# xuhao1/TaichiSLAM

Measured on AMD Instinct MI355X. Metric: depth-frames/s integrated (640x480->512^3 TSDF), higher is better.
Workload: dtype f16 storage / f32 + int64 fixed-point arithmetic; 1 GPU; BASELINE configs[1]: single 640x480 u16 depth stream (sphere room r=3 m, 1 deg/frame) -> DenseTSDF 512^3 / 2 cm, recast_step 2, max_ray 5 m; one stream+submap per GPU

## Files before the change

### taichislam_amd/csrc/tsl_integrate.hip

```cpp
#include "tsl_tsdf.hpp"
#include <hip/hip_ext.h>

namespace tsl {

#ifdef TSL_TIMING
#define TSL_T0() const int _wv = (blockIdx.x * (int)blockDim.x + (int)threadIdx.x) >> 6
#define TSL_TICK(F, k) do { long long _n = wall_clock64(); if (lane_id() == 0 && _wv < 16384) (F).dbg[_wv * 16 + (k)] = _n; } while (0)
#else
#define TSL_T0() do {} while (0)
#define TSL_TICK(F, k) do {} while (0)
#endif

#define SCATTER_TILE 4096

struct RayRegs { float pf0, pf1, pf2, d0, d1, d2, P0, P1, P2, w; long long qden; int n; };

__device__ __forceinline__ uint32_t wave_min_u32(uint32_t v)
{
    for (int d = 32; d > 0; d >>= 1) { const uint32_t o = (uint32_t)__shfl_xor((int)v, d); v = o < v ? o : v; }
    return v;
}
__device__ __forceinline__ RayRegs make_ray(const uint4 rec, int n, const FrameParams& P)
{
    RayRegs R;
// ... 527 lines not shown
#else
__device__ __forceinline__ int acc_swz5(int l) { return l ^ (((l >> 8) ^ (l >> 5)) & 31); }
#endif
struct StepK { float vs, rvs, T0, T1, T2; int hN, hNz; };

template <bool FASTDIV>
__device__ __forceinline__ void step_eval(const RayRegs& R, const StepK& K, int j, int* slot, float* qf)
{
    const float jf = (float)j;
    const float x0 = (R.d0 * jf) * K.vs + K.T0, x1 = (R.d1 * jf) * K.vs + K.T1, x2 = (R.d2 * jf) * K.vs + K.T2;
    const int i0 = rnd_i(div_vs(x0, K.vs, K.rvs, FASTDIV ? 1 : 0)), i1 = rnd_i(div_vs(x1, K.vs, K.rvs, FASTDIV ? 1 : 0)), i2 = rnd_i(div_vs(x2, K.vs, K.rvs, FASTDIV ? 1 : 0));
    *slot = acc_swz5((((i0 + K.hN) & 15) << 8) | (((i1 + K.hN) & 15) << 4) | ((i2 + K.hNz) & 15));
    const float v0 = R.P0 - x0, v1 = R.P1 - x1, v2 = R.P2 - x2;
    const float s2 = (v0 * v0 + v1 * v1) + v2 * v2;
    const float dist = sqrt_rn_norm(fmaxf(s2, 1.2621774483536189e-29f));
    const float dot = (v0 * R.pf0 + v1 * R.pf1) + v2 * R.pf2;
    const float sd = dot == 0.0f ? 0.0f : copysignf(dist, dot);
    *qf = rintf((R.w * sd) * TSL_FIX_SCALE);
}

__device__ __forceinline__ bool fits_i32(long long q) { return q == (long long)(int)q; }
__device__ __forceinline__ float from_fix32(long long q) { return (float)(int)q * (float)TSL_FIX_INV; }

#define FLUSH_CHUNK 4
template <int N>
__device__ __forceinline__ void apply_chunk(const uint32_t* old, const long long* qn, const long long* qd, uint32_t* nv, bool all_small)
{
    if (all_small) {
#pragma unroll
        for (int q = 0; q < N; ++q) nv[q] = apply_update_f(old[q], from_fix32(qn[q]), from_fix32(qd[q]));
    } else {
#pragma unroll
        for (int q = 0; q < N; ++q) nv[q] = apply_update_f(old[q], from_fix(qn[q]), from_fix(qd[q]));
    }
}

__device__ __forceinline__ int uni(int v) { return __builtin_amdgcn_readfirstlane(v); }
#define IT_UNIT 0
#define IT_POOL 1
#define IT_SLAB 2
#define IT_NP   3
#define IT_TMALL 4
#define IT_FMASK 5
#define IT_OFF  6
#define IT_N    (IT_OFF + TSL_NB)
#define IT_WORDS (IT_N + TSL_NB + 2)
#define NRANGE (PLAN_NCLS * (TSL_NB + 1))

template <bool TEX, bool FASTDIV, int NT, int SPT, int WPE>
__global__ void __launch_bounds__(NT, WPE) k_integrate_batch(MapDev M, BatchDev B, int kind)
{
    constexpr int CSEGS = SPT * NT, VPT = TSL_BRK3 / NT, CH = VPT < FLUSH_CHUNK ? VPT : FLUSH_CHUNK;
    static_assert(VPT <= 16, "the written / first-touch masks hold 16 voxels per thread");
#ifdef TSL_EXP_SLOT16
    __shared__ ulonglong2 s_acc[TSL_BRK3];
#define S_NUM(i) s_acc[i].x
#define S_DEN(i) s_acc[i].y
#else
    __shared__ unsigned long long s_num[TSL_BRK3];
    __shared__ unsigned long long s_den[TSL_BRK3];
#define S_NUM(i) s_num[i]
#define S_DEN(i) s_den[i]
#endif
    __shared__ unsigned long long s_keys[CSEGS];
    __shared__ uint32_t s_win[TEX ? TSL_BRK3 : 1];
    __shared__ int s_bin[64];
    __shared__ int s_claim[2];
    __shared__ int s_uq[TSL_NB];
    __shared__ int s_cum[NRANGE + 1];
    __shared__ int s_it[3][IT_WORDS];
    uint32_t okmask = 0u;
#pragma unroll
    for (int q = 0; q < TSL_NB; ++q) if (q < B.n) {
        const FrameDev& Fq = B.f[q];
        if (Fq.counters[HDR_FAIL] == 0) okmask |= 1u << q;
        const int nact = min(Fq.counters[1], Fq.max_frame_bricks);
        for (int i = blockIdx.x * NT + threadIdx.x; i < nact; i += gridDim.x * NT) { const int b = Fq.act_b[i]; Fq.bhist[b] = 0; Fq.bcursor[b] = 0; }
    }
    if (threadIdx.x < TSL_NB) s_uq[threadIdx.x] = 0;
    if (threadIdx.x == 0) {
        int acc = 0, k = 0;
#ifdef TSL_CLASS_MAJOR
        for (int c = 0; c < PLAN_NCLS; ++c) {
            s_cum[k++] = acc; acc += min(B.f[0].counters[HDR_UNITS + c], B.f[0].unit_cap);
            for (int q = 0; q < TSL_NB; ++q) { s_cum[k++] = acc; if ((okmask >> q) & 1u) acc += min(B.f[q].counters[HDR_PARTS + c], B.f[q].part_cap); }
        }
#else
        for (int c = 0; c < PLAN_NCLS; ++c) { s_cum[k++] = acc; if (kind != 2) acc += min(B.f[0].counters[HDR_UNITS + c], B.f[0].unit_cap); }
        for (int c = 0; c < PLAN_NCLS; ++c)
            for (int q = 0; q < TSL_NB; ++q) { s_cum[k++] = acc; if (kind != 1 && ((okmask >> q) & 1u)) acc += min(B.f[q].counters[HDR_PARTS + c], B.f[q].part_cap); }
#endif
        s_cum[NRANGE] = acc;
        s_claim[0] = __hip_atomic_fetch_add(&B.f[0].counters[kind == 2 ? HDR_CLAIM2 : HDR_CLAIM], 1, __ATOMIC_RELAXED, __HIP_MEMORY_SCOPE_AGENT);
    }
    __syncthreads();
    const int total = uni(s_cum[NRANGE]);
    int* const claim = &B.f[0].counters[kind == 2 ? HDR_CLAIM2 : HDR_CLAIM];
    auto entry_of = [&](int r, int* kq) -> int4 {
        int k = 0;
#pragma unroll
        for (int j = 1; j < NRANGE; ++j) k += r >= uni(s_cum[j]) ? 1 : 0;
#ifdef TSL_CLASS_MAJOR
// ... 23 lines not shown
            int pool = e.z;
            if (fm == 0u) { fm = 1u; pool = -1; }
            it[IT_UNIT] = kq < 0 ? 1 : 0; it[IT_POOL] = pool; it[IT_SLAB] = kq < 0 ? 0 : e.w; it[IT_NP] = kq < 0 ? 1 : (e.y >> 16) & ((1 << PART_NP_BITS) - 1);
            it[IT_TMALL] = (int)tm; it[IT_FMASK] = (int)fm;
        }
    };
    const int r0 = uni(s_claim[0]);
    if (r0 >= total) return;
    { int kq, io, in; const int4 e = entry_of(r0, &kq); info_of(e, kq, &io, &in); commit(0, e, kq, io, in); }
    __syncthreads();
    auto steps_of = [&](int sl, uint32_t fm) -> int {
        int n = 0;
#pragma unroll
        for (int q = 0; q < TSL_NB; ++q) if ((fm >> q) & 1u) n += max(1, (uni(s_it[sl][IT_N + q]) + CSEGS - 1) / CSEGS);
        return n;
    };
    long long uniq = 0;
    int t = 0, slot = 0, c = 0; (void)t;
    int n_known = 0;
    bool exhausted = false;
    int f = __builtin_ctz((uint32_t)uni(s_it[0][IT_FMASK]));

    unsigned long long kk[SPT]; uint4 recs[SPT]; uint32_t wids[SPT];
#define TSL_SORT_DEAL(KIN, NSEG, FD)                                                                                    \
    {                                                                                                                   \
        int rr[SPT];                                                                                                    \
        _Pragma("unroll") for (int q = 0; q < SPT; ++q) {                                                               \
            const int i = q * NT + (int)threadIdx.x; rr[q] = -1;                                                        \
            if (i < (NSEG)) rr[q] = atomicAdd(&s_bin[63 - (int)(KIN[q] & 63ull)], 1);                                   \
        }                                                                                                               \
        __syncthreads();                                                                                                \
        if (threadIdx.x < 64) {                                                                                         \
            const int cb = s_bin[threadIdx.x]; int inc = cb;                                                            \
            for (int d = 1; d < 64; d <<= 1) { const int o = __shfl_up(inc, d); if ((int)threadIdx.x >= d) inc += o; }  \
            s_bin[threadIdx.x] = inc - cb;                                                                              \
        }                                                                                                               \
        __syncthreads();                                                                                                \
        _Pragma("unroll") for (int q = 0; q < SPT; ++q) if (rr[q] >= 0) s_keys[s_bin[63 - (int)(KIN[q] & 63ull)] + rr[q]] = KIN[q]; \
        __syncthreads();                                                                                                \
        _Pragma("unroll") for (int q = 0; q < SPT; ++q) {                                                               \
            const int i = q * NT + ((q & 1) ? NT - 1 - (int)threadIdx.x : (int)threadIdx.x);                            \
            if (i < (NSEG)) {                                                                                           \
                kk[q] = s_keys[i];                                                                                      \
                const int r = (int)((kk[q] >> (SEG_CNT_BITS + SEG_J_BITS)) & ((1u << STG_RAY_BITS) - 1));               \
                recs[q] = (FD).rayA[r];                                                                                 \
                wids[q] = TEX ? (FD).rayFirst[r] + 1u : 0u;                                                             \
            }                                                                                                           \
        }                                                                                                               \
        if (threadIdx.x < 64) s_bin[threadIdx.x] = 0;               \
    }
#define TSL_PRIME(SL, FQ)                                                                                               \
    {                                                                                                                   \
        const FrameDev& F0 = B.f[FQ];                                                                                   \
        const int off0 = uni(s_it[SL][IT_OFF + (FQ)]), nseg0 = min(uni(s_it[SL][IT_N + (FQ)]), CSEGS);                  \
        unsigned long long k0[SPT];                                                                                     \
        _Pragma("unroll") for (int q = 0; q < SPT; ++q) { const int i = q * NT + threadIdx.x; k0[q] = i < nseg0 ? F0.seg_sorted[off0 + i] : 0ull; } \
        TSL_SORT_DEAL(k0, nseg0, F0)                                                                                    \
    }

    {
#ifdef TSL_EXP_SLOT16
        for (int i = threadIdx.x; i < TSL_BRK3; i += NT) s_acc[i] = make_ulonglong2(0ull, 0ull);
#else
        ulonglong2* zn = reinterpret_cast<ulonglong2*>(s_num); ulonglong2* zd = reinterpret_cast<ulonglong2*>(s_den);
        for (int i = threadIdx.x; i < TSL_BRK3 / 2; i += NT) { zn[i] = make_ulonglong2(0ull, 0ull); zd[i] = make_ulonglong2(0ull, 0ull); }
#endif
// ... 33 lines not shown
        if (threadIdx.x == 0 && first_step) { _ph[0] = _ph[1] = _ph[2] = _ph[3] = _ph[4] = 0; }
        const long long _ta = wall_clock64();
#endif
        const bool has_next = !last_step || n_known >= 1;
        int fx = f, cx = c + 1, slotx = slot;
        if (last_chunk) {
            cx = 0;
            if (!last_frame) fx = f + 1 + __builtin_ctz(later);
            else if (has_next) { slotx = slot1; fx = __builtin_ctz((uint32_t)uni(s_it[slotx][IT_FMASK])); }
        }
        const FrameDev& Fx = B.f[fx];
        unsigned long long kn[SPT];
        const int offx = uni(s_it[slotx][IT_OFF + fx]) + cx * CSEGS;
        const int nsegn = has_next ? min(CSEGS, uni(s_it[slotx][IT_N + fx]) - cx * CSEGS) : 0;
#pragma unroll
        for (int q = 0; q < SPT; ++q) { const int i = q * NT + threadIdx.x; kn[q] = i < nsegn ? Fx.seg_sorted[offx + i] : 0ull; }
        const uint32_t* const twr = M.tw + (size_t)(p >= 0 ? p : 0) * TSL_BRK3;
        if (first_step) { have_old = false; vmask = 0u; }
        if (!TEX && unit && p >= 0 && first_step) {
#pragma unroll
            for (int q = 0; q < VPT; ++q) old[q] = twr[q * NT + threadIdx.x];
            have_old = true;
        }
#pragma unroll
        for (int q = 0; q < SPT; ++q) {
            const int i = q * NT + ((q & 1) ? NT - 1 - (int)threadIdx.x : (int)threadIdx.x);
            if (i >= nseg) continue;
            const unsigned long long key = kk[q];
            const int cnt = (int)(key & ((1u << SEG_CNT_BITS) - 1)), j0 = (int)((key >> SEG_CNT_BITS) & ((1u << SEG_J_BITS) - 1));
            const RayRegs R = make_ray(recs[q], 0, P);
            const uint32_t wid = wids[q];
#ifndef TSL_EXP_STAGGER
#define TSL_EXP_STAGGER 27
#endif
            int off = ((int)((threadIdx.x * (unsigned)TSL_EXP_STAGGER) & 63u) * cnt) >> 6;
            for (int s = 0; s < cnt; s += 2) {
                const int ja = j0 + off; off = (off + 1 == cnt) ? 0 : off + 1;
                const int jb = j0 + off; off = (off + 1 == cnt) ? 0 : off + 1;
                int la, lb; float qa, qb;
                step_eval<FASTDIV>(R, K, ja, &la, &qa);
                step_eval<FASTDIV>(R, K, jb, &lb, &qb);
                long long na = (long long)(int)qa, nb = (long long)(int)qb;
                if (__builtin_expect(__any(!(fabsf(qa) < 2147483648.0f) || !(fabsf(qb) < 2147483648.0f)), 0)) { na = __float2ll_rn(qa); nb = __float2ll_rn(qb); }
                atomicAdd(&S_NUM(la), (unsigned long long)na);
                atomicAdd(&S_DEN(la), (unsigned long long)R.qden);
                if (TEX) atomicMax(&s_win[la], wid);
                const bool vb = s + 1 < cnt;
#ifdef TSL_EXP_ADDZERO
                atomicAdd(&S_NUM(lb), (unsigned long long)(vb ? nb : 0ll));
                atomicAdd(&S_DEN(lb), (unsigned long long)(vb ? R.qden : 0ll));
// ... 16 lines not shown
        }
        if (has_next) TSL_SORT_DEAL(kn, nsegn, Fx)
        if (fetching) info_of(ne, nkq, &nio, &nin);
#ifdef TSL_TIMING
        const long long _tc = wall_clock64();
        if (threadIdx.x == 0) { _ph[0] += _tb - _ta; _ph[1] += _tc - _tb; _ph[4] += 1; }
#endif
        if (!last_chunk) {
            if (fetching) { commit(n_known == 0 ? slot1 : slot2, ne, nkq, nio, nin); ++n_known; __syncthreads(); }
            ++c; continue;
        }
        if (p >= 0 && threadIdx.x == 0) M.touch[p] = 1;
        if (p >= 0 && unit) {
            uint32_t* tw = M.tw + (size_t)p * TSL_BRK3;
            if (!have_old) {
#pragma unroll
                for (int q = 0; q < VPT; ++q) old[q] = tw[q * NT + threadIdx.x];
                have_old = true;
            }
            if (first_frame) {
#pragma unroll
                for (int q = 0; q < VPT; ++q) vmask |= ((old[q] >> 16) == 0u ? 1u : 0u) << (16 + q);
            }
#pragma unroll
            for (int h = 0; h < VPT; h += CH) {
                long long qn[CH], qd[CH]; uint32_t nv[CH]; bool small = true, anyu = false;
#pragma unroll
                for (int q = 0; q < CH; ++q) {
                    const int ls = acc_swz5((h + q) * NT + threadIdx.x);
                    qn[q] = (long long)S_NUM(ls); qd[q] = (long long)S_DEN(ls); S_NUM(ls) = 0ull; S_DEN(ls) = 0ull;
                    small = small && fits_i32(qn[q]) && fits_i32(qd[q]); anyu = anyu || qd[q] != 0;
                }
                if (!__any(anyu)) continue;
                apply_chunk<CH>(old + h, qn, qd, nv, __all(small));
#pragma unroll
                for (int q = 0; q < CH; ++q) {
                    const bool upd = qd[q] != 0;
                    old[h + q] = upd ? nv[q] : old[h + q];
                    vmask |= (upd ? 1u : 0u) << (h + q);
                    uniq += upd ? 1 : 0;
                    if (TEX && upd) {
                        const int l = (h + q) * NT + threadIdx.x;
                        reinterpret_cast<uint2*>(M.col)[(size_t)p * TSL_BRK3 + l] = F.colpix[s_win[acc_swz5(l)] - 1u];
                    }
                }
            }
            if (TEX) for (int i = threadIdx.x; i < TSL_BRK3; i += NT) s_win[i] = 0u;
            if (last_frame) {
                int8_t* obs = M.obs + (size_t)p * TSL_BRK3;
#pragma unroll
                for (int q = 0; q < VPT; ++q) {
                    const int l = q * NT + threadIdx.x;
                    if ((vmask >> q) & 1u) {
                        tw[l] = old[q];
                        if ((vmask >> (16 + q)) & 1u) obs[l] = 1;
                    }
                }
            }
        } else if (p >= 0) {
            ulonglong2* acc = reinterpret_cast<ulonglong2*>(F.acc) + (size_t)rk * TSL_BRK3;
#pragma unroll
            for (int q = 0; q < VPT; ++q) {
                const int l = q * NT + threadIdx.x, ls = acc_swz5(l);
                acc[l] = make_ulonglong2(S_NUM(ls), S_DEN(ls));
                S_NUM(ls) = 0ull; S_DEN(ls) = 0ull;
                if (TEX) { F.accw[(size_t)rk * TSL_BRK3 + l] = s_win[ls]; s_win[ls] = 0u; }
            }
// ... 10 lines not shown
        const long long _td = wall_clock64();
#endif
        {
            const long long u = wave_sum_ll(uniq);
            if (lane_id() == 0 && u) atomicAdd(&s_uq[f], (int)u);
            uniq = 0;
        }
        if (fetching) { commit(n_known == 0 ? slot1 : slot2, ne, nkq, nio, nin); ++n_known; }
#ifdef TSL_TIMING
        if (threadIdx.x == 0 && last_step) _rec[4] = wall_clock64();
        if (threadIdx.x == 0) { _ph[2] += _td - _tc; _ph[3] += wall_clock64() - _td; }
#endif
        if (!has_next && n_known == 0) break;
        __syncthreads();
        c = 0;
        if (last_frame) { ++t; slot = slot1; --n_known; f = __builtin_ctz((uint32_t)uni(s_it[slot][IT_FMASK])); }
        else f = fx;
        if (!has_next) TSL_PRIME(slot, f)
    }
#undef TSL_PRIME
#undef TSL_SORT_DEAL
    __syncthreads();
    if (threadIdx.x < TSL_NB && s_uq[threadIdx.x]) atomic_add_i64(&B.f[threadIdx.x].stats->unique, (long long)s_uq[threadIdx.x]);
}

#ifndef APPLY_SPLIT
#define APPLY_SPLIT 8
#endif
#ifndef APPLY_ROUND
#define APPLY_ROUND 2
#endif
template <bool TEX>
__global__ void __launch_bounds__(256) k_apply_slab(MapDev M, BatchDev B)
{
    __shared__ int s_uq[TSL_NB];
    constexpr int VP = TSL_BRK3 / APPLY_SPLIT / 256;
    uint32_t okmask = 0u;
#pragma unroll
    for (int q = 0; q < TSL_NB; ++q) if (q < B.n && B.f[q].counters[HDR_FAIL] == 0) okmask |= 1u << q;
    const int nheavy = min(B.f[0].counters[HDR_HEAVY], B.f[0].max_frame_bricks);
    const ulonglong2* const slab = reinterpret_cast<const ulonglong2*>(B.f[0].acc);
    if (threadIdx.x < TSL_NB) s_uq[threadIdx.x] = 0;
    __syncthreads();
    for (int item = blockIdx.x; item < nheavy * APPLY_SPLIT; item += gridDim.x) {
        const int4 e = B.f[0].heavy_tab[item / APPLY_SPLIT];
        const int b = e.x, p = e.y;
// ... 83 lines not shown
int launch_segments(tsl_tsdf* m, const BatchDev& B, const FrameParams* hp, int total, hipStream_t st)
{
    const FrameParams& P = hp[0];
    if (P.variant != 2) return TSL_OK;
    const int iblocks = (int)(((int64_t)total * P.split + 255) / 256);
    prof_begin(m, TSL_K_SEGMENTS, st);
    if (P.group) hipLaunchKernelGGL(k_segments<true>, dim3(iblocks, B.n), dim3(256), 0, st, m->M, B);
    else hipLaunchKernelGGL(k_segments<false>, dim3(iblocks, B.n), dim3(256), 0, st, m->M, B);
    prof_end(m, st);
    int unit_max = m->unit_max <= m->unit_floor ? m->unit_max : std::max(m->unit_floor, (int)((long long)m->unit_max * B.n / TSL_NB));
    int unit_half = std::min(unit_max, m->unit_half <= 2048 ? m->unit_half : std::max(2048, (int)((long long)m->unit_half * B.n / TSL_NB)));
    if (P.seq && m->seq_impl) unit_max = unit_half = 1 << 30;
    prof_begin(m, TSL_K_BIN, st);
    hipLaunchKernelGGL(k_plan, dim3((B.f[0].max_frame_bricks + 255) / 256, B.n), dim3(256), 0, st, m->M, B, m->chunks * m->wg * m->spt, unit_max, unit_half);
    hipLaunchKernelGGL(k_scatter, dim3(256, B.n), dim3(256), 0, st, B);
    prof_end(m, st);
    return TSL_OK;
}

int launch_brick(tsl_tsdf* m, const BatchDev& B, const FrameParams& P, int kind, hipStream_t st, hipEvent_t start, hipEvent_t stop)
{
    const int bg = kind == 2 ? m->pgrid : (B.n <= 2 ? (m->bgrid + 1) / 2 : (kind == 1 ? m->ugrid : m->bgrid));
#define TSL_LAUNCH_IB(TEXV, FD) do { \
        if (m->wg == 512 && m->spt == 2 && !TEXV) hipExtLaunchKernelGGL((k_integrate_batch<false, FD, 512, 2, 4>), dim3((2 * m->ncu * bg + 99) / 100), dim3(512), 0, st, start, stop, 0, m->M, B, kind); \
        else if (m->wg == 512) hipExtLaunchKernelGGL((k_integrate_batch<TEXV, FD, 512, 4, 2>), dim3((m->ncu * bg + 99) / 100), dim3(512), 0, st, start, stop, 0, m->M, B, kind); \
        else hipExtLaunchKernelGGL((k_integrate_batch<TEXV, FD, 256, 4, (TEXV ? 1 : 2)>), dim3(((TEXV ? 1 : 2) * m->ncu * bg + 99) / 100), dim3(256), 0, st, start, stop, 0, m->M, B, kind); } while (0)
    if (P.tex) { if (P.fastdiv) TSL_LAUNCH_IB(true, true); else TSL_LAUNCH_IB(true, false); }
    else { if (P.fastdiv) TSL_LAUNCH_IB(false, true); else TSL_LAUNCH_IB(false, false); }
#undef TSL_LAUNCH_IB
    TSL_HIP(hipGetLastError());
    return TSL_OK;
}
int launch_slab_apply(tsl_tsdf* m, const BatchDev& B, const FrameParams& P)
{
    prof_begin(m, TSL_K_FINALIZE);
    if (P.tex) hipLaunchKernelGGL(k_apply_slab<true>, dim3(16 * m->ncu), dim3(256), 0, m->stream_, m->M, B);
    else hipLaunchKernelGGL(k_apply_slab<false>, dim3(16 * m->ncu), dim3(256), 0, m->stream_, m->M, B);
    prof_end(m);
    TSL_HIP(hipGetLastError());
    return TSL_OK;
}
int launch_apply_batch(tsl_tsdf* m, const BatchDev& B, const FrameParams& P, hipEvent_t start, hipEvent_t stop)
{
    const int rc = launch_brick(m, B, P, 0, m->stream_, start, stop);
    return rc ? rc : launch_slab_apply(m, B, P);
}

int launch_apply(tsl_tsdf* m, FSet& S, int total)
{
// ... 16 lines not shown
```

### taichislam_amd/csrc/tsl_tsdf.hip

```cpp
#include "tsl_tsdf.hpp"
#include <rocprim/rocprim.hpp>
#include <algorithm>
#include <cmath>
#include <cstdio>
#include <cstdlib>
#include <cstring>
#include <mutex>

namespace tsl {

static thread_local std::string g_err;
void set_error(const std::string& s) { g_err = s; }

__device__ __forceinline__ uint32_t part1by2_32(uint32_t x)
{
    x &= 0x3ffu;
    x = (x ^ (x << 16)) & 0xff0000ffu;
    x = (x ^ (x << 8)) & 0x0300f00fu;
    x = (x ^ (x << 4)) & 0x030c30c3u;
    x = (x ^ (x << 2)) & 0x09249249u;
    return x;
}
__device__ __forceinline__ uint64_t part1by2_64(uint64_t x)
{
// ... 857 lines not shown
    FrameParams& P = m->P; std::memset(&P, 0, sizeof(P));
    for (int i = 0; i < 3; ++i) P.R[i * 4] = 1.0f;
    P.vs = (float)cfg->voxel_scale;
    {
        const float y0 = (float)(1.0 / (double)P.vs);
        float best = y0; double err = std::fabs(1.0 - (double)y0 * (double)P.vs);
        const float cand[2] = { std::nextafterf(y0, 0.0f), std::nextafterf(y0, INFINITY) };
        for (float c : cand) { const double e = std::fabs(1.0 - (double)c * (double)P.vs); if (e < err) { err = e; best = c; } }
        P.rvs = best; P.fastdiv = 0;
    }
    P.thr_max = (float)(cfg->max_ray_length * 1000.0); P.thr_min = (float)(cfg->min_ray_length * 1000.0);
    P.max_ray_f = (float)cfg->max_ray_length;
    P.max_steps_f = (float)(cfg->max_ray_length / cfg->voxel_scale);
    P.internal_f = (float)cfg->internal_voxels;
    P.pcl_lo = m->pcl_lo; P.pcl_ext = m->pcl_ext; P.pcl_bits = m->pcl_bits; P.pcl_blk = blk; P.seq = 0;
    P.step = cfg->recast_step; P.same_proj = cfg->color_same_proj;
    m->surf_thres = (float)(cfg->voxel_scale * 1.8);
    m->disp_floor = (float)cfg->disp_floor; m->disp_ceiling = (float)cfg->disp_ceiling;
    m->baseR.assign((size_t)m->npose * 9, 0.0); m->baseT.assign((size_t)m->npose * 3, 0.0);
    m->baseRf.assign((size_t)m->npose * 9, 0.0f); m->baseTf.assign((size_t)m->npose * 3, 0.0f);
    for (int s = 0; s < m->npose; ++s) for (int i = 0; i < 3; ++i) { m->baseR[(size_t)s * 9 + i * 4] = 1.0; m->baseRf[(size_t)s * 9 + i * 4] = 1.0f; }
    std::memset(m->gbaseR, 0, sizeof(m->gbaseR)); std::memset(m->gbaseT, 0, sizeof(m->gbaseT));
    for (int i = 0; i < 3; ++i) m->gbaseR[i * 4] = 1.0;
    m->P.group = 1; m->phases = 3; m->wg = 512; m->spt = 2; m->adaptive = 0; m->ramp_batches = 2; m->ramp_size = 4; m->bgrid = 75; m->ugrid = 75; m->pgrid = 25; m->split_launch = 0; m->chunks = 4; m->unit_max = 1024 * TSL_NB; m->unit_half = 1 << 20; m->unit_floor = 4096; m->batch_gen = 0;
    { hipDeviceProp_t pr; TSL_HIP(hipGetDeviceProperties(&pr, device)); m->ncu = pr.multiProcessorCount > 0 ? pr.multiProcessorCount : 256; }
    m->active = 0; m->variant = 2; m->split = 2; m->semantics = 0; m->seq_impl = 1; m->seq_ready = false; m->seq_bytes0 = 0; m->seq_d = nullptr; m->seq_tuple_cap = 0;
    m->prof_on = false; m->prof_open = false; m->prof_group = false; m->prof_mask = ~0u; std::memset(m->prof_ms, 0, sizeof(m->prof_ms)); std::memset(m->prof_n, 0, sizeof(m->prof_n));
    m->sort_temp = nullptr; m->sort_temp_bytes = 0;
    m->xbuf = nullptr; m->xbuf_bytes = 0; m->mesh_v = m->mesh_n = m->mesh_c = nullptr; m->mesh_count = nullptr; m->mesh_cap = 0; m->mesh_flags = nullptr;
    m->fuse_acc = nullptr; m->fuse_cnt = nullptr; m->fuse_cacc = nullptr; m->fuse_dirty = false; m->mrg_nunion = -1;
    m->esdf = nullptr; m->esdf_par = nullptr; m->esdf_ok = nullptr; m->esdf_mode = 0; m->esdf_grid = 0; m->fuse_direct = false; m->merge_exchange = 0; m->mrg_racc = m->mrg_rcnt = m->mrg_rec = nullptr; m->mrg_racc_bytes = m->mrg_rcnt_bytes = m->mrg_rec_bytes = 0; m->esdf_orphans = 0; m->esdf_last = nullptr; m->esdf_in = nullptr; m->esdf_read = nullptr; m->esdf_overlap = true; m->esdf_ctr_idx = 0; for (int k = 0; k < 2; ++k) { m->fseq_keys[k] = m->fseq_vals[k] = nullptr; m->fseq_bytes[k] = m->fseq_vbytes[k] = 0; } m->fseq_temp = nullptr; m->fseq_tbytes = 0; m->fseq_ctr = nullptr; m->esdf_gate = nullptr; m->esdf_gate_ev = nullptr; m->esdf_gate_set = false; m->esdf_gate_mask = 0; m->esdf_valid = false; m->esdf_force_full = false; m->pose_dev = nullptr;

    MapDev& M = m->M; std::memset(&M, 0, sizeof(M));
    M.N = m->N; M.Nz = m->Nz; M.nbx = m->nbx; M.nbz = m->nbz; M.nb3 = m->nb3; M.nsub = m->nsub; M.hN = m->N / 2; M.hNz = m->Nz / 2;
    int64_t want = cfg->max_bricks > 0 ? cfg->max_bricks : 32768 * (int64_t)(m->nsub > 4 ? 4 : (m->nsub > 1 ? m->nsub : 1));
    const int64_t all = (int64_t)m->nsub * m->nb3;
    if (want > all) want = all;
    M.max_bricks = (int)want;
    int rc;
    if ((rc = dev_alloc(m, (void**)&M.table, sizeof(int) * (size_t)all, 0xff))) return rc;
    if ((rc = dev_alloc(m, (void**)&M.tw, sizeof(uint32_t) * (size_t)want * TSL_BRK3, 0))) return rc;
    if ((rc = dev_alloc(m, (void**)&M.obs, (size_t)want * TSL_BRK3, 0))) return rc;
    if ((rc = dev_alloc(m, (void**)&M.occ, (size_t)want * TSL_BRK3, 0))) return rc;
    if (cfg->texture_enabled) { if ((rc = dev_alloc(m, (void**)&M.col, sizeof(uint16_t) * 4 * (size_t)want * TSL_BRK3, 0))) return rc; }
    if ((rc = dev_alloc(m, (void**)&M.owner, sizeof(int) * (size_t)want, 0))) return rc;
    if ((rc = dev_alloc(m, (void**)&M.touch, (size_t)want, 0))) return rc;
    if ((rc = dev_alloc(m, (void**)&M.pool_top, sizeof(int) * 4, 0))) return rc;
// ... 138 lines not shown
    m->clean = true;
    return rc ? rc : ec;
}
int tsl_tsdf_memory_bytes(const tsl_tsdf* m, int64_t* b) { TSL_REQUIRE(m && b, "null"); *b = m->bytes; return TSL_OK; }

static int take_deferred(tsl_tsdf* m) { const int rc = m->deferred_rc; m->deferred_rc = 0; return rc; }
static int read_int(tsl_tsdf* m, const int* dev, int* out)
{
    TSL_HIP(hipMemcpyAsync(m->h_ints, dev, sizeof(int), hipMemcpyDeviceToHost, ms(m)));
    TSL_HIP(hipStreamSynchronize(ms(m)));
    *out = m->h_ints[0];
    return take_deferred(m);
}
static int check_dev_err(tsl_tsdf* m) { (void)ms(m); return take_dev_err(m); }
int tsl_tsdf_get_option(tsl_tsdf* m, const char* name, int* value)
{
    TSL_REQUIRE(m && name && value, "null");
    if (!std::strcmp(name, "group")) { *value = m->P.group; return TSL_OK; }
    if (!std::strcmp(name, "esdf_mode")) { *value = m->esdf_mode; return TSL_OK; }
    if (!std::strcmp(name, "fuse_window_misses")) { return read_int(m, m->M.pool_top + 2, value); }
    if (!std::strcmp(name, "esdf_orphans")) { int rc = esdf_finish(m); if (rc) return rc; *value = (int)m->esdf_orphans; return TSL_OK; }
    if (!std::strcmp(name, "semantics")) { *value = m->semantics; return TSL_OK; }
    if (!std::strcmp(name, "seq_impl")) { *value = m->seq_impl; return TSL_OK; }
    if (!std::strcmp(name, "last_heavy_bricks") || !std::strcmp(name, "last_slab_slots")) {
        TSL_REQUIRE(m->scratch_ready, "nothing integrated yet");
        int rc = tsl_tsdf_sync(m); if (rc) return rc;
        const int bi = (m->cur + TSL_NBATCH - 1) % TSL_NBATCH;
        int v[40];
        TSL_HIP(hipMemcpy(v, m->fset[bi * TSL_NB].F.counters, sizeof(v), hipMemcpyDeviceToHost));
        *value = name[5] == 'h' ? v[14] : v[13];
        return TSL_OK;
    }
    if (!std::strcmp(name, "seq_longest_run")) {
        TSL_REQUIRE(m->scratch_ready, "nothing integrated yet");
        int rc = tsl_tsdf_sync(m); if (rc) return rc;
        const int bi = (m->cur + TSL_NBATCH - 1) % TSL_NBATCH;
        long long sum = 0;
        for (int q = 0; q < m->last_batch_n; ++q) { int v[40]; TSL_HIP(hipMemcpy(v, m->fset[bi * TSL_NB + q].F.counters, sizeof(v), hipMemcpyDeviceToHost)); sum += (unsigned)v[31]; }
        *value = (int)(sum > 0x7fffffffll ? 0x7fffffffll : sum);
        return TSL_OK;
    }
    if (!std::strcmp(name, "seq_long_voxels")) {
        TSL_REQUIRE(m->scratch_ready, "nothing integrated yet");
        int rc = tsl_tsdf_sync(m); if (rc) return rc;
        const int bi = (m->cur + TSL_NBATCH - 1) % TSL_NBATCH;
        int v[40]; TSL_HIP(hipMemcpy(v, m->fset[bi * TSL_NB].F.counters, sizeof(v), hipMemcpyDeviceToHost));
        *value = v[28] + v[30];
#ifdef TSL_SEQ_DBG
        fprintf(stderr, "seq dbg (long role, last batch): evaluations %d, commits that moved T %d, commits that moved W only %d\n", v[32], v[33], v[34]);
#endif
        return TSL_OK;
    }
    if (!std::strcmp(name, "fastdiv")) { *value = m->P.fastdiv; return TSL_OK; }
// ... 388 lines not shown
                return rc;
            }
        }
        return TSL_OK;
    }
    if (!std::strcmp(name, "fastdiv")) { if (value == 0) m->P.fastdiv = 0; return TSL_OK; }
    if (!std::strcmp(name, "mesh_gather")) { m->mesh_gather = value != 0; return TSL_OK; }
    if (!std::strcmp(name, "esdf_full")) { m->esdf_force_full = value != 0; return TSL_OK; }
    if (!std::strcmp(name, "esdf_mode")) { TSL_REQUIRE(value == 0 || value == 1, "esdf_mode: 0 = regional recompute (default), 1 = raise / lower wavefront with parent directions"); int rc = esdf_finish(m); if (rc) return rc; m->esdf_mode = value; m->esdf_valid = false; return TSL_OK; }
    if (!std::strcmp(name, "esdf_round_cap")) { m->esdf_round_cap = value; return TSL_OK; }
    if (!std::strcmp(name, "merge_exchange")) { TSL_REQUIRE(value == 0 || value == 1, "merge_exchange: 0 = all-reduce of the packed sums, 1 = reduce-scatter + all-gather of finalised voxels"); m->merge_exchange = value; return TSL_OK; }
    if (!std::strcmp(name, "fuse_direct")) { m->fuse_direct = value != 0; return TSL_OK; }
    if (!std::strcmp(name, "esdf_grid")) { TSL_REQUIRE(value >= 0, "esdf_grid: workgroups of a relaxation round (0 = four per CU)"); m->esdf_grid = value; return TSL_OK; }
    if (!std::strcmp(name, "esdf_overlap")) { int rc = esdf_finish(m); if (rc) return rc; m->esdf_overlap = value != 0; return TSL_OK; }
    if (!std::strcmp(name, "unit")) { TSL_REQUIRE(value >= 0 && value <= (1 << 20), "unit must be 0..2^20 segments"); int rc = tsl_tsdf_sync(m); if (rc) return rc; m->unit_max = value; return TSL_OK; }
    if (!std::strcmp(name, "unit_floor")) { TSL_REQUIRE(value >= 0 && value <= (1 << 20), "unit_floor must be 0..2^20 segments"); int rc = tsl_tsdf_sync(m); if (rc) return rc; m->unit_floor = value; return TSL_OK; }
    if (!std::strcmp(name, "unit_half")) { TSL_REQUIRE(value >= 0 && value <= (1 << 20), "unit_half must be 0..2^20 segments"); int rc = tsl_tsdf_sync(m); if (rc) return rc; m->unit_half = value; return TSL_OK; }
    if (!std::strcmp(name, "chunks")) { TSL_REQUIRE(value >= 1 && value <= 8, "chunks must be 1..8"); int rc = tsl_tsdf_sync(m); if (rc) return rc; m->chunks = value; return TSL_OK; }
    if (!std::strcmp(name, "adaptive")) { m->adaptive = value != 0; return TSL_OK; }
    if (!std::strcmp(name, "ramp_size")) { TSL_REQUIRE(value >= 1 && value <= TSL_NB, "ramp_size must be 1..8 frames"); m->ramp_size = value; return TSL_OK; }
    if (!std::strcmp(name, "ramp")) { TSL_REQUIRE(value >= 0 && value <= 16, "ramp must be 0..16 half batches"); m->ramp_batches = value; return TSL_OK; }
    if (!std::strcmp(name, "ugrid") || !std::strcmp(name, "pgrid")) { TSL_REQUIRE(value >= 5 && value <= 200, "ugrid / pgrid must be 5..200 (percent of the resident workgroup slots)"); { int rc = tsl_tsdf_sync(m); if (rc) return rc; } (name[0] == 'u' ? m->ugrid : m->pgrid) = value; return TSL_OK; }
    if (!std::strcmp(name, "split_launch")) { TSL_REQUIRE(value == 0 || value == 1, "split_launch must be 0 or 1"); { int rc = tsl_tsdf_sync(m); if (rc) return rc; } m->split_launch = value; return TSL_OK; }
    if (!std::strcmp(name, "bgrid")) { TSL_REQUIRE(value >= 10 && value <= 200, "bgrid must be 10..200 (percent of the resident workgroup slots)"); { int rc = tsl_tsdf_sync(m); if (rc) return rc; } m->bgrid = value; return TSL_OK; }
    if (!std::strcmp(name, "spt")) { TSL_REQUIRE(value == 2 || value == 4, "spt must be 2 or 4"); { int rc = tsl_tsdf_sync(m); if (rc) return rc; } m->spt = value; return TSL_OK; }
    if (!std::strcmp(name, "wg")) { TSL_REQUIRE(value == 256 || value == 512, "wg must be 256 or 512"); { int rc = tsl_tsdf_sync(m); if (rc) return rc; } m->wg = value; return TSL_OK; }
    if (!std::strcmp(name, "phases")) { int rc = tsl_tsdf_sync(m); if (rc) return rc; m->phases = value & 3; return TSL_OK; }
    if (!std::strcmp(name, "overlap")) { int rc = tsl_tsdf_sync(m); if (rc) return rc; m->overlap = value < 0 ? 0 : (value > TSL_NB ? TSL_NB : value); for (auto& H : m->batch) H.b_pending = false; return TSL_OK; }
    if (!std::strcmp(name, "split")) { TSL_REQUIRE(value >= 1 && value <= 64 && (64 % value) == 0, "split must divide 64"); m->split = value; return TSL_OK; }
    set_error("unknown option"); return TSL_ERR_ARG;
}

}
```

### taichislam_amd/csrc/tsl_tsdf.hpp

```cpp
#pragma once
#include "tsl_common.hpp"

namespace tsl {

struct FrameParams {
    float R[9], T[3];
    float fx, fy, cx, cy;
    float fxc, fyc, cxc, cyc;
    float vs;
    float rvs; int fastdiv;
    float thr_max, thr_min;
    float max_ray_f;
    float max_steps_f;
    float internal_f;
    int   pcl_lo, pcl_ext, pcl_bits;
    int   step, hh, ww, H, W;
    int   rstride;
    int   cstride;
    int   th, tw, tex, same_proj;
    int   slot;
    int   variant, split;
    int   group;
    int   seq, pcl_blk;
    int   hlog2;
// ... 34 lines not shown

#define SEG_CNT_BITS 6
#define SEG_J_BITS   12
#define SEG_RAY_BITS 24
#define SEG_SLOT_SHIFT (SEG_CNT_BITS + SEG_J_BITS + SEG_RAY_BITS)
#define SEG_MAX_CNT 63
#define STG_RAY_BITS 22
#define STG_B_SHIFT (SEG_CNT_BITS + SEG_J_BITS + STG_RAY_BITS)
#define PART_NP_BITS 12
#define SLAB_SLOT_BITS 20
#define PLAN_NCLS 4
#define HDR_FAIL 11
#define HDR_CLAIM 12
#define HDR_SLAB 13
#define HDR_HEAVY 14
#define HDR_PARTS 16
#define HDR_UNITS 20
#define HDR_CLAIM2 24
#define HDR_SEQ_TUPLES 26
#define HDR_SEQ_LONG 28
#define HDR_SEQ_XLONG 30
#define HDR_SEQ_MAXRUN 31
#define HDR_SEQ_CLAIM 35
#define HDR_SEQ_SLOTS 29

__device__ __forceinline__ void frame_fail(const MapDev& M, const FrameDev& F, int bits) { atomicOr(&F.counters[11], bits); atomicOr(M.err, bits); }

#define H_INL 13
#define H_BLOCK_SHIFT 44
#define H_EMPTY 0ull
__device__ __forceinline__ unsigned long long h_key(unsigned long long vkey, int block) { return (vkey | ((unsigned long long)block << H_BLOCK_SHIFT)) + 1ull; }
#define GROUP_BIG_CAP 16384
struct HSlot { unsigned long long key; int cnt; uint32_t pix[H_INL]; };
static_assert(sizeof(HSlot) == 64, "one slot per 64 bytes");
__device__ __forceinline__ uint32_t h_hash64(unsigned long long key, int log2n) { return (uint32_t)((key * 0x9E3779B97F4A7C15ull) >> (64 - log2n)); }

struct PixAcc { int cnt; h16 sx, sy, sz, zs, cr, cg, cb; };

__device__ __forceinline__ void acc_colour(const FrameParams& P, const FrameDev& F, uint32_t pid, PixAcc& A)
{
    const uint8_t* rgb;
    if (P.points) rgb = P.tex_input + (size_t)pid * 3;
    else {
        const int jj = (int)pid / P.ww, ii = (int)pid - jj * P.ww;
        const int pj = jj * P.step, pi = ii * P.step;
        if (P.same_proj) rgb = P.tex_input + ((size_t)pj * P.tw + pi) * 3;
// ... 119 lines not shown
    uint32_t* mesh_flags;
    float *mesh_v, *mesh_n, *mesh_c; int* mesh_count; int64_t mesh_cap; int mesh_gather;
    void *fuse_acc, *fuse_cnt, *fuse_cacc; bool fuse_dirty;
    uint8_t* mrg_mask; int *mrg_list, *mrg_count; int mrg_nunion;
    void *mrg_pacc, *mrg_pcnt; size_t mrg_pacc_bytes, mrg_pcnt_bytes;
    void *mrg_racc, *mrg_rcnt, *mrg_rec; size_t mrg_racc_bytes, mrg_rcnt_bytes, mrg_rec_bytes; int merge_exchange;
    float* esdf; uint8_t *esdf_fl, *esdf_region, *esdf_par, *esdf_ok; int esdf_mode, esdf_grid; bool fuse_direct; long long esdf_orphans; int *esdf_list, *esdf_queue, *esdf_ctr, *esdf_inq, *esdf_nbr; uint32_t* esdf_note; int esdf_qcap;
    float *esdf_exp_xyz, *esdf_exp_val; int* esdf_exp_count; int esdf_exp_n;
    bool esdf_valid, esdf_force_full; int esdf_submap; float esdf_gamma, esdf_maxd; tsl_esdf_stats esdf_stats;
    bool esdf_query_ok; int* esdf_q_ctr; int esdf_q_rounds;
    hipEvent_t esdf_gate, esdf_gate_ev; bool esdf_gate_set; unsigned esdf_gate_mask;
    hipEvent_t esdf_in, esdf_read, esdf_last;
    bool esdf_overlap; int esdf_ctr_idx;
    void *fseq_keys[2], *fseq_vals[2], *fseq_temp; size_t fseq_bytes[2], fseq_vbytes[2], fseq_tbytes; void* fseq_ctr;
    EsdfSlot esdf_slot[TSL_ESDF_SLOTS]; int esdf_tail, esdf_npend, esdf_rounds_seen, esdf_round_cap; bool esdf_short; tsl_esdf_totals_t esdf_tot;
    bool prof_on, prof_open, prof_group; unsigned prof_mask; std::vector<tsl::ProfSlot> prof; std::vector<hipEvent_t> prof_free;
    double prof_ms[TSL_K_COUNT]; int64_t prof_n[TSL_K_COUNT];
    int semantics;
    int seq_impl;
    bool seq_ready; int64_t seq_bytes0;
    tsl::SeqDev seq_h[TSL_NSETS]; tsl::SeqDev* seq_d;
    void *seqb_keys[TSL_NBATCH][2], *seqb_vals[TSL_NBATCH][2], *seqb_temp[TSL_NBATCH], *seqb_long[TSL_NBATCH], *seqb_lmask[TSL_NBATCH], *seqb_perm[TSL_NBATCH]; size_t seqb_temp_bytes; long long seq_tuple_cap;
    unsigned long long *seq_keys[2], *seq_vals[2], *seq_ctr; void* seq_temp; size_t seq_temp_bytes; long long seq_cap;
    int variant, split, phases, wg, spt, ncu, chunks, unit_max, unit_half, unit_floor, bgrid, ugrid, pgrid, split_launch, adaptive, ramp, ramp_batches, ramp_size; bool clean; uint64_t batch_gen;
    int64_t bytes;
    void* seqv_sum[TSL_NBATCH]; int* seqv_log;
    uint32_t shape_hash; int dry_launches;
};

namespace tsl {
int  grow(void** p, size_t* have, size_t need);
hipStream_t ms(tsl_tsdf* m);
int  flush_pending(tsl_tsdf* m);
void prof_begin(tsl_tsdf* m, int kid, hipStream_t st = nullptr, int count = 1);
void prof_end(tsl_tsdf* m, hipStream_t st = nullptr);
bool prof_slot(tsl_tsdf* m, int kid, int count, hipEvent_t* a, hipEvent_t* b);
void convert_pose(const double* Rb, const double* Tb, const double* R, const double* T, float* outR, float* outT);
int  dev_alloc(tsl_tsdf* m, void** p, size_t bytes, int fill);
int  check_variant2(tsl_tsdf* m);
int  launch_segments(tsl_tsdf* m, const BatchDev& B, const FrameParams* hp, int total, hipStream_t st);
int  launch_apply(tsl_tsdf* m, FSet& S, int total);
int  launch_apply_batch(tsl_tsdf* m, const BatchDev& B, const FrameParams& P, hipEvent_t start = nullptr, hipEvent_t stop = nullptr);
int  launch_brick(tsl_tsdf* m, const BatchDev& B, const FrameParams& P, int kind, hipStream_t st, hipEvent_t start, hipEvent_t stop);
int  launch_slab_apply(tsl_tsdf* m, const BatchDev& B, const FrameParams& P);
int  launch_seq_group(tsl_tsdf* m, const BatchDev& B, const FrameParams* hp, int bi, hipStream_t st);
int  launch_seq_apply(tsl_tsdf* m, const BatchDev& B, const FrameParams& P, int bi);
void seq_release(tsl_tsdf* m);
// ... 8 lines not shown
```

Baseline: 34160 frames/s.

## Split ray segments across idle threads when deal is underfilled; per-voxel flush

When a sorted batch of ray segments fills at most half (or a quarter, or an eighth) of the workgroup's segment slots, each segment is cut into 2, 4 or 8 contiguous pieces so idle threads share the per-ray stepping work. Pieces are built by rewriting the count and start fields of the packed key. The shared-accumulator flush is also reworked from 4-voxel chunks to per-voxel handling that first reads all denominators and then skips untouched voxels wave-wide. This adds per-block counters recording how often each split factor is used, plus one extra atomic per block. The change is on by default and can be switched off through a new deal_split knob.

After: 33970 frames/s. About the same (-0.6%).

```diff
diff --git a/taichislam_amd/csrc/tsl_deal_split.h b/taichislam_amd/csrc/tsl_deal_split.h
--- /dev/null
+++ b/taichislam_amd/csrc/tsl_deal_split.h
@@ -0,0 +1,39 @@
+#ifndef TSL_DEAL_SPLIT_H
+#define TSL_DEAL_SPLIT_H
+
+#if defined(__HIPCC__)
+#define TSL_DS_HD __host__ __device__ __forceinline__
+#else
+#define TSL_DS_HD inline
+#endif
+
+namespace tsl {
+
+#define TSL_DS_CNT_BITS 6
+#define TSL_DS_J_BITS 12
+
+TSL_DS_HD int deal_split_log2(int nseg, int csegs)
+{
+    if (nseg <= 0) return 0;
+    return nseg * 8 <= csegs ? 3 : (nseg * 4 <= csegs ? 2 : (nseg * 2 <= csegs ? 1 : 0));
+}
+
+TSL_DS_HD unsigned long long deal_split_piece(unsigned long long key, int p, int lk)
+{
+    const int cnt = (int)(key & ((1u << TSL_DS_CNT_BITS) - 1)), j0 = (int)((key >> TSL_DS_CNT_BITS) & ((1u << TSL_DS_J_BITS) - 1));
+    const int base = cnt >> lk, r = cnt & ((1 << lk) - 1);
+    const int len = base + (p < r ? 1 : 0);
+    const int first = len ? j0 + p * base + (p < r ? p : r) : j0;
+    return (key & ~((1ull << (TSL_DS_CNT_BITS + TSL_DS_J_BITS)) - 1ull)) | ((unsigned long long)first << TSL_DS_CNT_BITS) | (unsigned long long)len;
+}
+
+}
+
+#endif
+
+#ifdef TSL_DEAL_SPLIT_C_API
+extern "C" {
+int tsl_deal_split_log2(int nseg, int csegs) { return tsl::deal_split_log2(nseg, csegs); }
+unsigned long long tsl_deal_split_piece(unsigned long long key, int p, int lk) { return tsl::deal_split_piece(key, p, lk); }
+}
+#endif
diff --git a/taichislam_amd/csrc/tsl_integrate.hip b/taichislam_amd/csrc/tsl_integrate.hip
--- a/taichislam_amd/csrc/tsl_integrate.hip
+++ b/taichislam_amd/csrc/tsl_integrate.hip
@@ -1,4 +1,5 @@
 #include "tsl_tsdf.hpp"
+#include "tsl_deal_split.h"
 #include <hip/hip_ext.h>
 
 namespace tsl {
@@ -573,7 +574,6 @@
 __device__ __forceinline__ bool fits_i32(long long q) { return q == (long long)(int)q; }
 __device__ __forceinline__ float from_fix32(long long q) { return (float)(int)q * (float)TSL_FIX_INV; }
 
-#define FLUSH_CHUNK 4
 template <int N>
 __device__ __forceinline__ void apply_chunk(const uint32_t* old, const long long* qn, const long long* qd, uint32_t* nv, bool all_small)
 {
@@ -599,9 +599,9 @@
 #define NRANGE (PLAN_NCLS * (TSL_NB + 1))
 
 template <bool TEX, bool FASTDIV, int NT, int SPT, int WPE>
-__global__ void __launch_bounds__(NT, WPE) k_integrate_batch(MapDev M, BatchDev B, int kind)
-{
-    constexpr int CSEGS = SPT * NT, VPT = TSL_BRK3 / NT, CH = VPT < FLUSH_CHUNK ? VPT : FLUSH_CHUNK;
+__global__ void __launch_bounds__(NT, WPE) k_integrate_batch(MapDev M, BatchDev B, int kind, int deal_split)
+{
+    constexpr int CSEGS = SPT * NT, VPT = TSL_BRK3 / NT;
     static_assert(VPT <= 16, "the written / first-touch masks hold 16 voxels per thread");
 #ifdef TSL_EXP_SLOT16
     __shared__ ulonglong2 s_acc[TSL_BRK3];
@@ -618,6 +618,7 @@
     __shared__ int s_bin[64];
     __shared__ int s_claim[2];
     __shared__ int s_uq[TSL_NB];
+    __shared__ int s_dk[4];
     __shared__ int s_cum[NRANGE + 1];
     __shared__ int s_it[3][IT_WORDS];
     uint32_t okmask = 0u;
@@ -629,6 +630,7 @@
         for (int i = blockIdx.x * NT + threadIdx.x; i < nact; i += gridDim.x * NT) { const int b = Fq.act_b[i]; Fq.bhist[b] = 0; Fq.bcursor[b] = 0; }
     }
     if (threadIdx.x < TSL_NB) s_uq[threadIdx.x] = 0;
+    if (threadIdx.x < 4) s_dk[threadIdx.x] = 0;
     if (threadIdx.x == 0) {
         int acc = 0, k = 0;
 #ifdef TSL_CLASS_MAJOR
@@ -698,6 +700,7 @@
     int f = __builtin_ctz((uint32_t)uni(s_it[0][IT_FMASK]));
 
     unsigned long long kk[SPT]; uint4 recs[SPT]; uint32_t wids[SPT];
+    auto split_lk = [&](int nseg) -> int { return deal_split ? deal_split_log2(nseg, CSEGS) : 0; };
 #define TSL_SORT_DEAL(KIN, NSEG, FD)                                                                                    \
     {                                                                                                                   \
         int rr[SPT];                                                                                                    \
@@ -714,10 +717,11 @@
         __syncthreads();                                                                                                \
         _Pragma("unroll") for (int q = 0; q < SPT; ++q) if (rr[q] >= 0) s_keys[s_bin[63 - (int)(KIN[q] & 63ull)] + rr[q]] = KIN[q]; \
         __syncthreads();                                                                                                \
+        const int lk_ = split_lk(NSEG);                                                                                 \
         _Pragma("unroll") for (int q = 0; q < SPT; ++q) {                                                               \
             const int i = q * NT + ((q & 1) ? NT - 1 - (int)threadIdx.x : (int)threadIdx.x);                            \
-            if (i < (NSEG)) {                                                                                           \
-                kk[q] = s_keys[i];                                                                                      \
+            if (i < ((NSEG) << lk_)) {                                                                                  \
+                kk[q] = deal_split_piece(s_keys[i >> lk_], i & ((1 << lk_) - 1), lk_);                                  \
                 const int r = (int)((kk[q] >> (SEG_CNT_BITS + SEG_J_BITS)) & ((1u << STG_RAY_BITS) - 1));               \
                 recs[q] = (FD).rayA[r];                                                                                 \
                 wids[q] = TEX ? (FD).rayFirst[r] + 1u : 0u;                                                             \
@@ -797,10 +801,12 @@
             for (int q = 0; q < VPT; ++q) old[q] = twr[q * NT + threadIdx.x];
             have_old = true;
         }
+        const int ndealt = nseg << split_lk(nseg);
+        if (threadIdx.x == 0) s_dk[split_lk(nseg)] += 1;
 #pragma unroll
         for (int q = 0; q < SPT; ++q) {
             const int i = q * NT + ((q & 1) ? NT - 1 - (int)threadIdx.x : (int)threadIdx.x);
-            if (i >= nseg) continue;
+            if (i >= ndealt) continue;
             const unsigned long long key = kk[q];
             const int cnt = (int)(key & ((1u << SEG_CNT_BITS) - 1)), j0 = (int)((key >> SEG_CNT_BITS) & ((1u << SEG_J_BITS) - 1));
             const RayRegs R = make_ray(recs[q], 0, P);
@@ -863,27 +869,23 @@
 #pragma unroll
                 for (int q = 0; q < VPT; ++q) vmask |= ((old[q] >> 16) == 0u ? 1u : 0u) << (16 + q);
             }
-#pragma unroll
-            for (int h = 0; h < VPT; h += CH) {
-                long long qn[CH], qd[CH]; uint32_t nv[CH]; bool small = true, anyu = false;
-#pragma unroll
-                for (int q = 0; q < CH; ++q) {
-                    const int ls = acc_swz5((h + q) * NT + threadIdx.x);
-                    qn[q] = (long long)S_NUM(ls); qd[q] = (long long)S_DEN(ls); S_NUM(ls) = 0ull; S_DEN(ls) = 0ull;
-                    small = small && fits_i32(qn[q]) && fits_i32(qd[q]); anyu = anyu || qd[q] != 0;
-                }
-                if (!__any(anyu)) continue;
-                apply_chunk<CH>(old + h, qn, qd, nv, __all(small));
-#pragma unroll
-                for (int q = 0; q < CH; ++q) {
-                    const bool upd = qd[q] != 0;
-                    old[h + q] = upd ? nv[q] : old[h + q];
-                    vmask |= (upd ? 1u : 0u) << (h + q);
-                    uniq += upd ? 1 : 0;
-                    if (TEX && upd) {
-                        const int l = (h + q) * NT + threadIdx.x;
-                        reinterpret_cast<uint2*>(M.col)[(size_t)p * TSL_BRK3 + l] = F.colpix[s_win[acc_swz5(l)] - 1u];
-                    }
+            long long qdv[VPT]; int lsv[VPT];
+#pragma unroll
+            for (int q = 0; q < VPT; ++q) { lsv[q] = acc_swz5(q * NT + threadIdx.x); qdv[q] = (long long)S_DEN(lsv[q]); }
+#pragma unroll
+            for (int q = 0; q < VPT; ++q) {
+                const bool upd = qdv[q] != 0;
+                if (!__any(upd)) continue;
+                const long long qn = (long long)S_NUM(lsv[q]);
+                if (upd) { S_NUM(lsv[q]) = 0ull; S_DEN(lsv[q]) = 0ull; }
+                uint32_t nv;
+                apply_chunk<1>(old + q, &qn, qdv + q, &nv, __all(fits_i32(qn) && fits_i32(qdv[q])));
+                old[q] = upd ? nv : old[q];
+                vmask |= (upd ? 1u : 0u) << q;
+                uniq += upd ? 1 : 0;
+                if (TEX && upd) {
+                    const int l = q * NT + threadIdx.x;
+                    reinterpret_cast<uint2*>(M.col)[(size_t)p * TSL_BRK3 + l] = F.colpix[s_win[lsv[q]] - 1u];
                 }
             }
             if (TEX) for (int i = threadIdx.x; i < TSL_BRK3; i += NT) s_win[i] = 0u;
@@ -940,6 +942,7 @@
 #undef TSL_SORT_DEAL
     __syncthreads();
     if (threadIdx.x < TSL_NB && s_uq[threadIdx.x]) atomic_add_i64(&B.f[threadIdx.x].stats->unique, (long long)s_uq[threadIdx.x]);
+    if (threadIdx.x < 4 && s_dk[threadIdx.x]) atomicAdd(&B.f[0].counters[HDR_DEAL + threadIdx.x], s_dk[threadIdx.x]);
 }
 
 #ifndef APPLY_SPLIT
@@ -1069,9 +1072,9 @@
 {
     const int bg = kind == 2 ? m->pgrid : (B.n <= 2 ? (m->bgrid + 1) / 2 : (kind == 1 ? m->ugrid : m->bgrid));
 #define TSL_LAUNCH_IB(TEXV, FD) do { \
-        if (m->wg == 512 && m->spt == 2 && !TEXV) hipExtLaunchKernelGGL((k_integrate_batch<false, FD, 512, 2, 4>), dim3((2 * m->ncu * bg + 99) / 100), dim3(512), 0, st, start, stop, 0, m->M, B, kind); \
-        else if (m->wg == 512) hipExtLaunchKernelGGL((k_integrate_batch<TEXV, FD, 512, 4, 2>), dim3((m->ncu * bg + 99) / 100), dim3(512), 0, st, start, stop, 0, m->M, B, kind); \
-        else hipExtLaunchKernelGGL((k_integrate_batch<TEXV, FD, 256, 4, (TEXV ? 1 : 2)>), dim3(((TEXV ? 1 : 2) * m->ncu * bg + 99) / 100), dim3(256), 0, st, start, stop, 0, m->M, B, kind); } while (0)
+        if (m->wg == 512 && m->spt == 2 && !TEXV) hipExtLaunchKernelGGL((k_integrate_batch<false, FD, 512, 2, 4>), dim3((2 * m->ncu * bg + 99) / 100), dim3(512), 0, st, start, stop, 0, m->M, B, kind, m->deal_split); \
+        else if (m->wg == 512) hipExtLaunchKernelGGL((k_integrate_batch<TEXV, FD, 512, 4, 2>), dim3((m->ncu * bg + 99) / 100), dim3(512), 0, st, start, stop, 0, m->M, B, kind, m->deal_split); \
+        else hipExtLaunchKernelGGL((k_integrate_batch<TEXV, FD, 256, 4, (TEXV ? 1 : 2)>), dim3(((TEXV ? 1 : 2) * m->ncu * bg + 99) / 100), dim3(256), 0, st, start, stop, 0, m->M, B, kind, m->deal_split); } while (0)
     if (P.tex) { if (P.fastdiv) TSL_LAUNCH_IB(true, true); else TSL_LAUNCH_IB(true, false); }
     else { if (P.fastdiv) TSL_LAUNCH_IB(false, true); else TSL_LAUNCH_IB(false, false); }
 #undef TSL_LAUNCH_IB
diff --git a/taichislam_amd/csrc/tsl_tsdf.hip b/taichislam_amd/csrc/tsl_tsdf.hip
--- a/taichislam_amd/csrc/tsl_tsdf.hip
+++ b/taichislam_amd/csrc/tsl_tsdf.hip
@@ -903,7 +903,7 @@
     for (int s = 0; s < m->npose; ++s) for (int i = 0; i < 3; ++i) { m->baseR[(size_t)s * 9 + i * 4] = 1.0; m->baseRf[(size_t)s * 9 + i * 4] = 1.0f; }
     std::memset(m->gbaseR, 0, sizeof(m->gbaseR)); std::memset(m->gbaseT, 0, sizeof(m->gbaseT));
     for (int i = 0; i < 3; ++i) m->gbaseR[i * 4] = 1.0;
-    m->P.group = 1; m->phases = 3; m->wg = 512; m->spt = 2; m->adaptive = 0; m->ramp_batches = 2; m->ramp_size = 4; m->bgrid = 75; m->ugrid = 75; m->pgrid = 25; m->split_launch = 0; m->chunks = 4; m->unit_max = 1024 * TSL_NB; m->unit_half = 1 << 20; m->unit_floor = 4096; m->batch_gen = 0;
+    m->P.group = 1; m->phases = 3; m->wg = 512; m->spt = 2; m->adaptive = 0; m->ramp_batches = 2; m->ramp_size = 4; m->bgrid = 75; m->ugrid = 75; m->pgrid = 25; m->split_launch = 0; m->deal_split = 1; m->chunks = 4; m->unit_max = 1024 * TSL_NB; m->unit_half = 1 << 20; m->unit_floor = 4096; m->batch_gen = 0;
     { hipDeviceProp_t pr; TSL_HIP(hipGetDeviceProperties(&pr, device)); m->ncu = pr.multiProcessorCount > 0 ? pr.multiProcessorCount : 256; }
     m->active = 0; m->variant = 2; m->split = 2; m->semantics = 0; m->seq_impl = 1; m->seq_ready = false; m->seq_bytes0 = 0; m->seq_d = nullptr; m->seq_tuple_cap = 0;
     m->prof_on = false; m->prof_open = false; m->prof_group = false; m->prof_mask = ~0u; std::memset(m->prof_ms, 0, sizeof(m->prof_ms)); std::memset(m->prof_n, 0, sizeof(m->prof_n));
@@ -1088,13 +1088,15 @@
     if (!std::strcmp(name, "esdf_orphans")) { int rc = esdf_finish(m); if (rc) return rc; *value = (int)m->esdf_orphans; return TSL_OK; }
     if (!std::strcmp(name, "semantics")) { *value = m->semantics; return TSL_OK; }
     if (!std::strcmp(name, "seq_impl")) { *value = m->seq_impl; return TSL_OK; }
-    if (!std::strcmp(name, "last_heavy_bricks") || !std::strcmp(name, "last_slab_slots")) {
+    if (!std::strcmp(name, "deal_split")) { *value = m->deal_split; return TSL_OK; }
+    if (!std::strcmp(name, "last_heavy_bricks") || !std::strcmp(name, "last_slab_slots") ||
+        !std::strcmp(name, "last_deal_k1") || !std::strcmp(name, "last_deal_k2") || !std::strcmp(name, "last_deal_k4") || !std::strcmp(name, "last_deal_k8")) {
         TSL_REQUIRE(m->scratch_ready, "nothing integrated yet");
         int rc = tsl_tsdf_sync(m); if (rc) return rc;
         const int bi = (m->cur + TSL_NBATCH - 1) % TSL_NBATCH;
         int v[40];
         TSL_HIP(hipMemcpy(v, m->fset[bi * TSL_NB].F.counters, sizeof(v), hipMemcpyDeviceToHost));
-        *value = name[5] == 'h' ? v[14] : v[13];
+        *value = name[5] == 'h' ? v[HDR_HEAVY] : (name[5] == 's' ? v[HDR_SLAB] : v[HDR_DEAL + (name[11] == '1' ? 0 : (name[11] == '2' ? 1 : (name[11] == '4' ? 2 : 3)))]);
         return TSL_OK;
     }
     if (!std::strcmp(name, "seq_longest_run")) {
@@ -1529,6 +1531,7 @@
     if (!std::strcmp(name, "ramp")) { TSL_REQUIRE(value >= 0 && value <= 16, "ramp must be 0..16 half batches"); m->ramp_batches = value; return TSL_OK; }
     if (!std::strcmp(name, "ugrid") || !std::strcmp(name, "pgrid")) { TSL_REQUIRE(value >= 5 && value <= 200, "ugrid / pgrid must be 5..200 (percent of the resident workgroup slots)"); { int rc = tsl_tsdf_sync(m); if (rc) return rc; } (name[0] == 'u' ? m->ugrid : m->pgrid) = value; return TSL_OK; }
     if (!std::strcmp(name, "split_launch")) { TSL_REQUIRE(value == 0 || value == 1, "split_launch must be 0 or 1"); { int rc = tsl_tsdf_sync(m); if (rc) return rc; } m->split_launch = value; return TSL_OK; }
+    if (!std::strcmp(name, "deal_split")) { TSL_REQUIRE(value == 0 || value == 1, "deal_split must be 0 or 1"); { int rc = tsl_tsdf_sync(m); if (rc) return rc; } m->deal_split = value; return TSL_OK; }
     if (!std::strcmp(name, "bgrid")) { TSL_REQUIRE(value >= 10 && value <= 200, "bgrid must be 10..200 (percent of the resident workgroup slots)"); { int rc = tsl_tsdf_sync(m); if (rc) return rc; } m->bgrid = value; return TSL_OK; }
     if (!std::strcmp(name, "spt")) { TSL_REQUIRE(value == 2 || value == 4, "spt must be 2 or 4"); { int rc = tsl_tsdf_sync(m); if (rc) return rc; } m->spt = value; return TSL_OK; }
     if (!std::strcmp(name, "wg")) { TSL_REQUIRE(value == 256 || value == 512, "wg must be 256 or 512"); { int rc = tsl_tsdf_sync(m); if (rc) return rc; } m->wg = value; return TSL_OK; }
diff --git a/taichislam_amd/csrc/tsl_tsdf.hpp b/taichislam_amd/csrc/tsl_tsdf.hpp
--- a/taichislam_amd/csrc/tsl_tsdf.hpp
+++ b/taichislam_amd/csrc/tsl_tsdf.hpp
@@ -80,6 +80,7 @@
 #define HDR_SEQ_XLONG 30
 #define HDR_SEQ_MAXRUN 31
 #define HDR_SEQ_CLAIM 35
+#define HDR_DEAL 36
 #define HDR_SEQ_SLOTS 29
 
 __device__ __forceinline__ void frame_fail(const MapDev& M, const FrameDev& F, int bits) { atomicOr(&F.counters[11], bits); atomicOr(M.err, bits); }
@@ -245,7 +246,7 @@
     tsl::SeqDev seq_h[TSL_NSETS]; tsl::SeqDev* seq_d;
     void *seqb_keys[TSL_NBATCH][2], *seqb_vals[TSL_NBATCH][2], *seqb_temp[TSL_NBATCH], *seqb_long[TSL_NBATCH], *seqb_lmask[TSL_NBATCH], *seqb_perm[TSL_NBATCH]; size_t seqb_temp_bytes; long long seq_tuple_cap;
     unsigned long long *seq_keys[2], *seq_vals[2], *seq_ctr; void* seq_temp; size_t seq_temp_bytes; long long seq_cap;
-    int variant, split, phases, wg, spt, ncu, chunks, unit_max, unit_half, unit_floor, bgrid, ugrid, pgrid, split_launch, adaptive, ramp, ramp_batches, ramp_size; bool clean; uint64_t batch_gen;
+    int variant, split, phases, wg, spt, ncu, chunks, unit_max, unit_half, unit_floor, bgrid, ugrid, pgrid, split_launch, deal_split, adaptive, ramp, ramp_batches, ramp_size; bool clean; uint64_t batch_gen;
     int64_t bytes;
     void* seqv_sum[TSL_NBATCH]; int* seqv_log;
     uint32_t shape_hash; int dry_launches;
```
